# matajoh/fourier_feature_nets

Measured on AMD Instinct MI355X. Metric: rays/sec (train), higher is better.
Workload: dtype f32

## Files before the change

fourier_feature_nets_amd/csrc/fourier_features.h:

```cpp
#pragma once
#include "common.h"

namespace ffn {

typedef float f32x4 __attribute__((ext_vector_type(4)));

struct EncRegs {
    const float* tab;
    int F;
    int raw;
    float scale;
};

__device__ __forceinline__ EncRegs load_enc(const ffn_encoding& e, const float* table) {
    EncRegs r;
    r.F = e.num_freq;
    r.tab = table;
    r.raw = (e.include_input != 0 || e.num_freq == 0) ? 1 : 0;
    r.scale = e.scale;
    return r;
}

typedef ffn_f32x2 f32x2;

template <bool TRIG_ONLY>
__device__ __forceinline__ f32x4 feature_quad(const EncRegs& enc, int g, int h, float x0, float x1,
                                              float x2, f32x2 s0, f32x2 s1, f32x2 s2) {
    const int k = 4 * g + 2 * h;
    const int kk = TRIG_ONLY ? k : (k < kEncRowPitch - 2 ? k : kEncRowPitch - 2);
    const f32x2 b0 = *reinterpret_cast<const f32x2*>(enc.tab + kk);
    const f32x2 b1 = *reinterpret_cast<const f32x2*>(enc.tab + kEncRowPitch + kk);
    const f32x2 b2 = *reinterpret_cast<const f32x2*>(enc.tab + 2 * kEncRowPitch + kk);
    const f32x2 amp = *reinterpret_cast<const f32x2*>(enc.tab + 3 * kEncRowPitch + kk);
    f32x2 ang = b0 * s0;
    ang = __builtin_elementwise_fma(s1, b1, ang);
    ang = __builtin_elementwise_fma(s2, b2, ang);
    f32x2 sn, cs;
    fast_sincos_n<f32x2, 2>(ang, sn, cs);
    const f32x2 c = amp * cs, s = amp * sn;
    f32x4 v;
    if (TRIG_ONLY) {
        v[0] = c[0]; v[1] = s[0]; v[2] = c[1]; v[3] = s[1];
        return v;
    }
#pragma unroll
    for (int j = 0; j < 2; ++j) {
        const int off = 2 * (k + j - enc.F);
        const float raw_even = (enc.raw && off == 0) ? x0 : ((enc.raw && off == 2) ? x2 : 0.0f);
        const float raw_odd = (enc.raw && off == 0) ? x1 : 0.0f;
        const bool trig = k + j < enc.F;
        v[2 * j] = trig ? c[j] : raw_even;
        v[2 * j + 1] = trig ? s[j] : raw_odd;
    }
    return v;
}

__device__ __forceinline__ void feature_oct(const EncRegs& enc, int g, int h, f32x4 s0, f32x4 s1,
                                            f32x4 s2, f32x4& va, f32x4& vb) {
    const float* t = enc.tab + 4 * g + 2 * h;
    auto two = [](const float* p) {
        const f32x2 lo = *reinterpret_cast<const f32x2*>(p), hi = *reinterpret_cast<const f32x2*>(p + 4);
        f32x4 v; v[0] = lo[0]; v[1] = lo[1]; v[2] = hi[0]; v[3] = hi[1];
        return v;
    };
    const f32x4 b0 = two(t), b1 = two(t + kEncRowPitch), b2 = two(t + 2 * kEncRowPitch);
    const f32x4 amp = two(t + 3 * kEncRowPitch);
    f32x4 ang = b0 * s0;
    ang = __builtin_elementwise_fma(s1, b1, ang);
    ang = __builtin_elementwise_fma(s2, b2, ang);
    f32x4 sn, cs;
    fast_sincos_n<f32x4, 4>(ang, sn, cs);
    const f32x4 c = amp * cs, s = amp * sn;
    va[0] = c[0]; va[1] = s[0]; va[2] = c[1]; va[3] = s[1];
    vb[0] = c[2]; vb[1] = s[2]; vb[2] = c[3]; vb[3] = s[3];
}

}
```

fourier_feature_nets_amd/csrc/mlp.hip:

```cpp
#include "fourier_features.h"
#include "composite_terms.h"
#include "focus_terms.h"
#include "occupancy_map.h"

namespace ffn {

typedef float f32x4 __attribute__((ext_vector_type(4)));
typedef f32x4 __attribute__((address_space(3))) lds_f32x4;
__device__ __forceinline__ lds_f32x4* lds_slab(const char* generic_lds_address) {
    return (lds_f32x4*)(uint32_t)(uintptr_t)generic_lds_address;
}
typedef float f32x16 __attribute__((ext_vector_type(16)));

constexpr int kSamplesPerWave = 32;
constexpr int kWavesPerBlock = 4;
constexpr int kActBytesPerWave = 32 * 1024;
constexpr int kBiasLdsFloats = 4096;

enum Mode { kInfer = 0, kTrainFwd = 1, kBackward = 2 };

__global__ void __launch_bounds__(256)
pack_kernel(const float* __restrict__ src, int rows, int cols, int ld, int transpose,
            const int32_t* __restrict__ row_map, const int32_t* __restrict__ col_map, int groups,
            int tiles, float* __restrict__ dst) {
    const int64_t total = (int64_t)groups * tiles * 256;
    for (int64_t e = (int64_t)blockIdx.x * blockDim.x + threadIdx.x; e < total;
         e += (int64_t)gridDim.x * blockDim.x) {
        const int p = (int)(e & 3);
        const int lane = (int)((e >> 2) & 63);
        const int64_t go = e >> 8;
        const int o = (int)(go % tiles);
        const int g = (int)(go / tiles);
        int r = 32 * o + (lane & 31);
        int c = 8 * g + 4 * (lane >> 5) + p;
        if (row_map != nullptr) r = row_map[r];
// ... 22 lines not shown
    }
    const int64_t total = (int64_t)job.groups * job.tiles * 256;
    for (int64_t e = (int64_t)blockIdx.x * blockDim.x + threadIdx.x; e < total;
         e += (int64_t)gridDim.x * blockDim.x) {
        const int p = (int)(e & 3);
        const int lane = (int)((e >> 2) & 63);
        const int64_t go = e >> 8;
        const int o = (int)(go % job.tiles);
        const int g = (int)(go / job.tiles);
        const int r = 32 * o + (lane & 31);
        int c = 8 * g + 4 * (lane >> 5) + p;
        if (job.col_map != nullptr) c = job.col_map[c];
        float v = 0.0f;
        if (c >= 0) {
            const int sr = job.transpose ? c : r;
            const int sc = job.transpose ? r : c;
            if (sr < job.rows && sc < job.cols) v = job.src[(int64_t)sr * job.ld + sc];
        }
        job.dst[e] = v;
    }
}

template <bool SAVE>
__device__ __forceinline__ void generate_features(const EncRegs& enc, int c0, int count, int h,
                                                  int s, int lane, float x0, float x1, float x2,
                                                  lds_f32x4* act, f32x4* fsave, int g_begin, int g_step) {
    const f32x2 s0 = (f32x2)(enc.scale * x0), s1 = (f32x2)(enc.scale * x1), s2 = (f32x2)(enc.scale * x2);
    const f32x4 q0 = (f32x4)(enc.scale * x0), q1 = (f32x4)(enc.scale * x1), q2 = (f32x4)(enc.scale * x2);
    int g_trig = (enc.F >> 2) - c0;
    g_trig = g_trig < 0 ? 0 : (g_trig > count ? count : g_trig);
    g_trig &= ~3;
    for (int g = g_begin; g < count; g += g_step) {
        f32x4 v[4];
        if (g < g_trig) {
            feature_oct(enc, c0 + g, h, q0, q1, q2, v[0], v[1]);
            feature_oct(enc, c0 + g + 2, h, q0, q1, q2, v[2], v[3]);
        } else {
#pragma unroll
            for (int u = 0; u < 4; ++u) v[u] = feature_quad<false>(enc, c0 + g + u, h, x0, x1, x2, s0, s1, s2);
        }
#pragma unroll
        for (int u = 0; u < 4; ++u) {
            act[(g + u) * 64 + lane] = v[u];
            if (SAVE) __builtin_nontemporal_store(v[u], &fsave[(2 * (c0 + g + u) + h) * 32 + (s ^ ((2 * (c0 + g + u) + h) & 15))]);
        }
    }
}

template <int OT>
__device__ __forceinline__ void mma_group(f32x16 (&acc)[OT], const f32x4 (&a)[OT], f32x4 x) {
#pragma unroll
    for (int p = 0; p < 4; ++p)
#pragma unroll
        for (int o = 0; o < OT; ++o)
            acc[o] = __builtin_amdgcn_mfma_f32_32x32x2f32(a[o][p], x[p], acc[o], 0, 0, 0);
}

template <int OT>
__device__ __forceinline__ void pipeline_plain() {
    __builtin_amdgcn_sched_group_barrier(0x020, 2 * OT, 0);
    __builtin_amdgcn_sched_group_barrier(0x100, 2, 0);
    __builtin_amdgcn_sched_group_barrier(0x008, 8 * OT, 0);
}
template <int OT, bool SAVES = false>
__device__ __forceinline__ void pipeline_spread() {
    __builtin_amdgcn_sched_group_barrier(0x100, 2, 0);
    if (SAVES) __builtin_amdgcn_sched_group_barrier(0x040, 2, 0);
#pragma unroll
    for (int i = 0; i < 2 * OT; ++i) {
        __builtin_amdgcn_sched_group_barrier(0x008, 4, 0);
        __builtin_amdgcn_sched_group_barrier(0x020, 1, 0);
    }
}
template <int OT>
__device__ __forceinline__ void load_group(f32x4 (&a)[OT], const f32x4* __restrict__ wg, int lane) {
    typedef const f32x4 __attribute__((address_space(1)))* gptr;
    const gptr lo = (gptr)wg;
    gptr hi = (gptr)(wg + 4 * 64);
    if (OT > 4) asm volatile("" : "+s"(hi));
#pragma unroll
    for (int o = 0; o < OT; ++o) a[o] = (o < 4 ? lo : hi)[(o & 3) * 64 + lane];
}

struct WaveCtx {
    int lane, h, s;
    float x0, x1, x2;
    float v0, v1, v2;
    f32x4 dl;
    lds_f32x4* act;
    const float* enc_table;
    const float* bias_lds;
    const float* bias_glb;
    uint4* masks;
    int64_t block;
    int64_t num_blocks;
    int64_t slab_block0;
    int64_t slab_blocks;
    float logit[4];
    int half;
    bool active;
};

__device__ __forceinline__ int saved_index(int cq, int s) { return cq * 32 + (s ^ (cq & 15)); }

__device__ __forceinline__ f32x4* slab_block(const ffn_mlp_chain& ch, float* base, int slot,
                                             const WaveCtx& w) {
    return reinterpret_cast<f32x4*>(base + ch.slot_offset[slot] * w.slab_blocks * 32) +
           (w.slab_block0 + w.block) * (int64_t)(ch.slot_channels[slot] * 8);
}

__device__ __forceinline__ void team_barrier() {
    asm volatile("s_waitcnt lgkmcnt(0)" ::: "memory");
    __builtin_amdgcn_s_barrier();
}

template <int OT, int MODE, int TWP, int FLAV, bool BIG = false>
__device__ __forceinline__ void run_step(const ffn_mlp_chain& ch, const ffn_step& L,
                                         const ffn_step* next, WaveCtx& w,
                                         const float* __restrict__ packed_w,
                                         f32x4 (&pre)[16],
                                         float* __restrict__ slab_out) {
    constexpr bool WIDE = TWP > 1;
    constexpr int TW = TWP;
    constexpr int kChunk = BIG ? 128 : (WIDE ? 64 : 32);
    const int half = WIDE ? w.half : 0;
    f32x16 acc[OT];
    if (MODE == kBackward) {
#pragma unroll
        for (int o = 0; o < OT; ++o)
#pragma unroll
            for (int r = 0; r < 16; ++r) acc[o][r] = 0.0f;
    } else if (L.b_off + 32 * OT * TW <= kBiasLdsFloats) {
        const float* bv = w.bias_lds + L.b_off + 32 * OT * half + 4 * w.h;
#pragma unroll
        for (int o = 0; o < OT; ++o)
#pragma unroll
            for (int q = 0; q < 4; ++q) {
                const f32x4 b4 = *reinterpret_cast<const f32x4*>(bv + 32 * o + 8 * q);
#pragma unroll
                for (int p = 0; p < 4; ++p) acc[o][4 * q + p] = b4[p];
            }
    } else {
        const float* bv = w.bias_glb + L.b_off + 32 * OT * half + 4 * w.h;
#pragma unroll
        for (int o = 0; o < OT; ++o)
#pragma unroll
            for (int q = 0; q < 4; ++q) {
                const f32x4 b4 = *reinterpret_cast<const f32x4*>(bv + 32 * o + 8 * q);
#pragma unroll
                for (int p = 0; p < 4; ++p) acc[o][4 * q + p] = b4[p];
            }
    }

    const f32x4* wp = reinterpret_cast<const f32x4*>(packed_w + L.w_off) + half * OT * 64;
    const int GA = L.act_groups;
    const int GX = L.aux_groups;
    const int G = GA + GX;
    constexpr int kGroupStride = TW * OT * 64;
    f32x4 wa0[OT], wa1[OT], wb0[OT], wb1[OT];
    f32x4 x0, x1, x2, x3;
#pragma unroll
    for (int o = 0; o < OT; ++o) { wa0[o] = pre[o]; wa1[o] = pre[8 + o]; }
    int gnext = 2;
    const int glast = G - 2;
    const f32x4* wnext = wp + 2 * kGroupStride;
    const int64_t mask_at = (((int64_t)(L.mask_slot < 0 ? 0 : L.mask_slot) * w.num_blocks + w.block) * TW + half) * 64 + w.lane;
    uint4 mbits = make_uint4(0xffffffffu, 0xffffffffu, 0xffffffffu, 0xffffffffu);
    if (MODE == kBackward && L.mask_slot >= 0) mbits = w.masks[mask_at];

    constexpr bool kTripSaves = MODE == kTrainFwd && !WIDE;
    const int feat_chunks = MODE == kBackward ? 0 : (GX + kChunk - 1) / kChunk;
    const int segs = (GA > 0 ? 1 : 0) + feat_chunks;
    for (int sg = 0; sg < segs; ++sg) {
        const bool feat = !(GA > 0 && sg == 0);
        int count = GA;
        f32x4* save = nullptr;
        if (!feat) {
            if (kTripSaves || (MODE != kInfer && L.save_in_slot >= 0 && w.active))
                save = slab_block(ch, slab_out, L.save_in_slot, w);
        } else {
            const int c0 = (sg - (GA > 0 ? 1 : 0)) * kChunk;
            count = GX - c0 < kChunk ? GX - c0 : kChunk;
            const EncRegs enc = load_enc(ch.enc[L.enc_id], w.enc_table + L.enc_id * kEncTablePitch);
            const float p0 = L.enc_id == 0 ? w.x0 : w.v0;
            const float p1 = L.enc_id == 0 ? w.x1 : w.v1;
            const float p2 = L.enc_id == 0 ? w.x2 : w.v2;
            if (WIDE && sg > 0) team_barrier();
            if (kTripSaves) {
                generate_features<false>(enc, c0, count, w.h, w.s, w.lane, p0, p1, p2, w.act, nullptr,
                                         4 * half, 4 * TW);
                save = slab_block(ch, slab_out, L.save_enc_slot, w) + c0 * 64;
            } else if (MODE == kTrainFwd && L.save_enc_slot >= 0 && w.active) {
                generate_features<true>(enc, c0, count, w.h, w.s, w.lane, p0, p1, p2, w.act,
                                        slab_block(ch, slab_out, L.save_enc_slot, w), 4 * half, 4 * TW);
            } else {
                generate_features<false>(enc, c0, count, w.h, w.s, w.lane, p0, p1, p2, w.act, nullptr,
                                         4 * half, 4 * TW);
            }
            if (WIDE) team_barrier();
        }
        const bool saving = MODE != kInfer && save != nullptr;
        const bool save_0 = saving && (TW == 1 || half == 0);
        const bool save_1 = saving && (TW == 1 || half == (TW == 2 ? 0 : 1));
        const bool save_2 = saving && (TW == 1 || half == (TW == 2 ? 1 : 2));
        const bool save_3 = saving && (TW == 1 || half == (TW == 2 ? 1 : 3));
        const unsigned save_lane = (unsigned)(w.h * 512 + ((w.s ^ w.h) << 4));
        char* save_s = reinterpret_cast<char*>(save);
#define FFN_SAVE(g, value)                                                                     \
    __builtin_nontemporal_store((value), reinterpret_cast<f32x4*>(save_s + (int64_t)(g) * 1024 +   \
                              (save_lane ^ (unsigned)((((g) * 2) & 15) << 4))))
        const lds_f32x4* xa = w.act + w.lane;
        x0 = xa[0];
        x1 = xa[64];
        if (MODE == kInfer || kTripSaves) {
            for (int g = 0; g < count; g += 4) {
                load_group<OT>(wb0, wnext, w.lane);
                load_group<OT>(wb1, wnext + kGroupStride, w.lane);
                x2 = xa[128];
                x3 = xa[192];
// ... 57 lines not shown
        f32x4 d = w.dl;
        f32x4 sel;
#pragma unroll
        for (int p = 0; p < 4; ++p) {
            float v = 0.0f;
#pragma unroll
            for (int c = 0; c < 4; ++c) v = (c == L.lg_col + p && p < L.lg_n) ? d[c] : v;
            sel[p] = w.h == 0 ? v : 0.0f;
        }
        mma_group<OT>(acc, wa0, sel);
    }

    const int ot_next = next != nullptr ? next->out_tiles / TW : 0;
    const f32x4* wn = next != nullptr
        ? reinterpret_cast<const f32x4*>(packed_w + next->w_off) + half * ot_next * 64 + w.lane
        : nullptr;

    f32x4* save_out = nullptr;
    if (MODE != kInfer && L.save_out_slot >= 0 && w.active) save_out = slab_block(ch, slab_out, L.save_out_slot, w);
    const bool fused_head = FLAV == 0 ? (MODE != kBackward && L.head_off >= 0)
                                      : (MODE != kBackward && FLAV >= 2);
    const bool to_slab = FLAV == 0 ? L.dst == 0 : true;
    const bool save_y = FLAV == 0 ? save_out != nullptr : FLAV == 2;
    const float* head_base = BIG ? w.bias_glb : w.bias_lds;
    const float* hw = head_base + (fused_head ? L.head_off : 0) + 4 + 16 * w.h;
    if (fused_head && w.h == 0 && half == 0) {
        const f32x4 hb = *reinterpret_cast<const f32x4*>(head_base + L.head_off);
#pragma unroll
        for (int c = 0; c < 4; ++c) w.logit[c] += hb[c];
    }
    if (WIDE) team_barrier();
    int e_lane = w.lane, e_h = w.h, e_s = w.s;
    if (WIDE) asm volatile("" : "+v"(e_lane), "+v"(e_h), "+v"(e_s));
    unsigned sign_bits[4] = {0u, 0u, 0u, 0u};
    const int relu_floor = L.relu ? 0 : (int)0x80000000;
#pragma unroll
    for (int o = 0; o < 8; ++o) {
        if (o < ot_next) {
            pre[o] = wn[o * 64];
            pre[8 + o] = wn[(int64_t)(TW * ot_next + o) * 64];
        }
        if (o >= OT) continue;
#pragma unroll
        for (int q = 0; q < 4; ++q) {
            const int group = 4 * (OT * half + o) + q;
            f32x4 y;
            if (MODE == kBackward) {
                const unsigned word = o < 2 ? mbits.x : (o < 4 ? mbits.y : (o < 6 ? mbits.z : mbits.w));
#pragma unroll
                for (int p = 0; p < 4; ++p) {
                    const int filled = ((OT & 1) && o == OT - 1) ? 16 : 32;
                    const int bit = filled - 1 - (16 * (o & 1) + 4 * q + p);
                    const int keep = ((int)(word << (31 - bit))) >> 31;
                    const float a = acc[o][4 * q + p];
                    y[p] = __builtin_bit_cast(float, __builtin_bit_cast(int, a) & keep);
                }
                w.act[group * 64 + e_lane] = y;
                if (save_y) __builtin_nontemporal_store(y, &save_out[saved_index(2 * group + e_h, e_s)]);
            } else {
                f32x4 hw4[4];
                if (fused_head) {
#pragma unroll
                    for (int p = 0; p < 4; ++p) hw4[p] = *reinterpret_cast<const f32x4*>(hw + group * 32 + p * 4);
                }
#pragma unroll
                for (int p = 0; p < 4; ++p) {
                    float t = acc[o][4 * q + p];
                    if (MODE == kTrainFwd)
                        sign_bits[o >> 1] = __builtin_amdgcn_alignbit(sign_bits[o >> 1],
                                                                      __builtin_bit_cast(unsigned, 0.0f - t), 31);
                    y[p] = __builtin_bit_cast(float, __builtin_elementwise_max(__builtin_bit_cast(int, t), relu_floor));
                }
                if (to_slab) {
                    w.act[group * 64 + e_lane] = y;
                    if (fused_head) {
#pragma unroll
                        for (int p = 0; p < 4; ++p) {
#pragma unroll
                            for (int c = 0; c < 4; ++c) w.logit[c] = __builtin_fmaf(y[p], hw4[p][c], w.logit[c]);
                        }
                        if (MODE == kTrainFwd && save_y) __builtin_nontemporal_store(y, &save_out[saved_index(2 * group + e_h, e_s)]);
                    }
                } else if (!WIDE && o == 0 && q == 0) {
#pragma unroll
                    for (int c = 0; c < 4; ++c) {
                        const int p = c - L.out_col;
// ... 41 lines not shown
                else run_step<8, MODE, TWP, 1, BIG>(ch, L, next, w, packed_w, pre, slab_out);
            } else if (!head && L.dst == 0) run_step<8, MODE, TWP, 1, BIG>(ch, L, next, w, packed_w, pre, slab_out);
            else run_step<8, MODE, TWP, 0, BIG>(ch, L, next, w, packed_w, pre, slab_out);
        } else if ((TWP < 4 || BIG) && ot == 4) run_step<4, MODE, TWP, 0, BIG>(ch, L, next, w, packed_w, pre, slab_out);
        else if (ot == 2) run_step<2, MODE, TWP, 0, BIG>(ch, L, next, w, packed_w, pre, slab_out);
        else run_step<1, MODE, TWP, 0, BIG>(ch, L, next, w, packed_w, pre, slab_out);
    }
}

constexpr int kTeamScratchBytes = 3072;

template <int TWP>
__device__ __forceinline__ void wave_setup(WaveCtx& w, char* smem, int64_t n, int64_t& stride) {
    constexpr bool WIDE = TWP > 1;
    w.lane = threadIdx.x & 63;
    w.h = w.lane >> 5;
    w.s = w.lane & 31;
    const int wave_in_block = __builtin_amdgcn_readfirstlane(threadIdx.x >> 6);
    const int teams = kWavesPerBlock / TWP;
    const int team = wave_in_block / TWP;
    w.half = WIDE ? (wave_in_block % TWP) : 0;
    stride = (int64_t)gridDim.x * teams;
    w.act = lds_slab(smem + team * (kActBytesPerWave * kWavesPerBlock / teams));
    w.enc_table = reinterpret_cast<const float*>(smem + kWavesPerBlock * kActBytesPerWave);
    w.bias_lds = reinterpret_cast<const float*>(smem + kWavesPerBlock * kActBytesPerWave + kEncTableBytes);
    w.num_blocks = (n + kSamplesPerWave - 1) / kSamplesPerWave;
    w.block = (int64_t)blockIdx.x * teams + team;
    w.slab_block0 = 0;
    w.slab_blocks = w.num_blocks;
    w.active = true;
}

template <int MODE, int TWP, bool BIG = false>
__global__ void __launch_bounds__(256, 1)
mlp_forward_kernel(const ffn_mlp_chain ch, const float* __restrict__ packed_w,
                   const float* __restrict__ bias, const float* __restrict__ positions,
                   const float* __restrict__ views, int64_t n, float* __restrict__ logits,
                   float* __restrict__ saved, uint32_t* __restrict__ masks, int64_t slab_block0,
                   int64_t slab_blocks) {
    extern __shared__ __attribute__((aligned(16))) char smem[];
    stage_encoding_tables(ch.enc, reinterpret_cast<float*>(smem + kWavesPerBlock * kActBytesPerWave),
                          threadIdx.x, 256);
    {
        float* bl = reinterpret_cast<float*>(smem + kWavesPerBlock * kActBytesPerWave + kEncTableBytes);
        const int staged = ch.bias_floats < kBiasLdsFloats ? ch.bias_floats : kBiasLdsFloats;
        for (int i = threadIdx.x; i < staged; i += 256) bl[i] = bias[i];
    }
    __syncthreads();
    constexpr bool WIDE = TWP > 1;
    WaveCtx w;
    int64_t stride;
    wave_setup<TWP>(w, smem, n, stride);
    w.bias_glb = bias;
    if (slab_blocks > 0) { w.slab_block0 = slab_block0; w.slab_blocks = slab_blocks; }
    w.masks = reinterpret_cast<uint4*>(masks);
    f32x4* scratch = reinterpret_cast<f32x4*>(smem + kWavesPerBlock * kActBytesPerWave + kEncTableBytes +
                                              kBiasLdsFloats * 4) + ((threadIdx.x >> 6) / TWP) * (TWP - 1) * 64;
    const int64_t passes = WIDE ? (w.num_blocks + stride - 1) / stride : 0;
    const int64_t first = w.block;
    float in_next[6] = {0.f, 0.f, 0.f, 0.f, 0.f, 0.f};
    auto request_inputs = [&](int64_t block) {
        block = block < w.num_blocks ? block : w.num_blocks - 1;
        const int64_t sample = block * kSamplesPerWave + w.s;
        const int64_t src = sample < n ? sample : n - 1;
        in_next[0] = positions[src * 3 + 0]; in_next[1] = positions[src * 3 + 1]; in_next[2] = positions[src * 3 + 2];
        if (views != nullptr) {
            in_next[3] = views[src * 3 + 0]; in_next[4] = views[src * 3 + 1]; in_next[5] = views[src * 3 + 2];
        }
    };
    request_inputs(first);
    for (int64_t pass = 0; WIDE ? pass < passes : w.block < w.num_blocks; ++pass) {
        if (WIDE) {
            w.block = first + pass * stride;
            w.active = w.block < w.num_blocks;
            if (!w.active) w.block = w.num_blocks - 1;
        }
// ... 29 lines not shown
    const uint32_t* occ_bits; GridMap map;
    float* color; float* alpha; float* depth; int32_t* nan_flag;
    uint8_t* image; int64_t pixel_offset;
};

constexpr int kRenderScratchBytes = 4096;

template <bool WIDE>
__global__ void __launch_bounds__(256, 1)
render_fused_kernel(const ffn_mlp_chain ch, const float* __restrict__ packed_w,
                    const float* __restrict__ bias, const RenderParams p) {
    extern __shared__ __attribute__((aligned(16))) char smem[];
    stage_encoding_tables(ch.enc, reinterpret_cast<float*>(smem + kWavesPerBlock * kActBytesPerWave),
                          threadIdx.x, 256);
    {
        float* bl = reinterpret_cast<float*>(smem + kWavesPerBlock * kActBytesPerWave + kEncTableBytes);
        const int staged = ch.bias_floats < kBiasLdsFloats ? ch.bias_floats : kBiasLdsFloats;
        for (int i = threadIdx.x; i < staged; i += 256) bl[i] = bias[i];
    }
    __syncthreads();
    WaveCtx w;
    int64_t stride;
    wave_setup<(WIDE ? 2 : 1)>(w, smem, kSamplesPerWave, stride);
    w.bias_glb = bias;
    w.block = 0;
    w.masks = nullptr;
    const int wave_in_block = __builtin_amdgcn_readfirstlane(threadIdx.x >> 6);
    constexpr int kTeams = WIDE ? 2 : kWavesPerBlock;
    const int team = WIDE ? wave_in_block >> 1 : wave_in_block;
    char* scratch = smem + kWavesPerBlock * kActBytesPerWave + kEncTableBytes + kBiasLdsFloats * 4;
    f32x4* partial = reinterpret_cast<f32x4*>(scratch) + team * 64;
    uint16_t* slots = reinterpret_cast<uint16_t*>(scratch + (WIDE ? 2048 : 0)) + team * 256;
    volatile int* team_blocks = reinterpret_cast<volatile int*>(scratch + 3072);
    const int S = p.S;
    const int rays_per_round = gridDim.x * kTeams;
    const int rounds = (p.num_rays + rays_per_round - 1) / rays_per_round;
    for (int round = 0; round < rounds; ++round) {
        const int r = WIDE ? (round * (int)gridDim.x + (int)blockIdx.x) * 2 + team
                           : (int)blockIdx.x * kWavesPerBlock + team + round * rays_per_round;
        bool have = r < p.num_rays;
        const int rr = have ? r : 0;
        const int64_t ray = p.ray_index != nullptr ? p.ray_index[rr] : p.ray_base + rr;
        if (have && p.valid != nullptr && p.valid[ray] == 0) {
            if (w.lane == 0 && w.half == 0) {
                if (p.color != nullptr) {
                    p.color[(int64_t)r * 3 + 0] = 0.f; p.color[(int64_t)r * 3 + 1] = 0.f;
                    p.color[(int64_t)r * 3 + 2] = 0.f;
                }
                if (p.alpha != nullptr) p.alpha[r] = 0.f;
                if (p.depth != nullptr) p.depth[r] = 0.f;
            }
            have = false;
        }
        if (!WIDE && !have) continue;
        const float sx = p.starts[ray * 3 + 0], sy = p.starts[ray * 3 + 1], sz = p.starts[ray * 3 + 2];
        const float dx = p.dirs[ray * 3 + 0], dy = p.dirs[ray * 3 + 1], dz = p.dirs[ray * 3 + 2];
// ... 92 lines not shown

struct FocusParams {
    const float* starts; const float* dirs; const float* near_far; int64_t total_rays;
    const int64_t* ray_index; int num_rays; int S; int n_focus;
    const float* unit_focus; const float* u; float* t_io;
};

template <bool WIDE>
__global__ void __launch_bounds__(256, 1)
focus_fused_kernel(const ffn_mlp_chain ch, const float* __restrict__ packed_w,
                   const float* __restrict__ bias, const FocusParams p) {
    extern __shared__ __attribute__((aligned(16))) char smem[];
    stage_encoding_tables(ch.enc, reinterpret_cast<float*>(smem + kWavesPerBlock * kActBytesPerWave),
                          threadIdx.x, 256);
    {
        float* bl = reinterpret_cast<float*>(smem + kWavesPerBlock * kActBytesPerWave + kEncTableBytes);
        const int staged = ch.bias_floats < kBiasLdsFloats ? ch.bias_floats : kBiasLdsFloats;
        for (int i = threadIdx.x; i < staged; i += 256) bl[i] = bias[i];
    }
    __syncthreads();
    WaveCtx w;
    int64_t stride;
    wave_setup<(WIDE ? 2 : 1)>(w, smem, kSamplesPerWave, stride);
    w.bias_glb = bias;
    w.block = 0;
    w.masks = nullptr;
    const int wave_in_block = __builtin_amdgcn_readfirstlane(threadIdx.x >> 6);
    constexpr int kTeams = WIDE ? 2 : kWavesPerBlock;
    const int team = WIDE ? wave_in_block >> 1 : wave_in_block;
    f32x4* partial = reinterpret_cast<f32x4*>(smem + kWavesPerBlock * kActBytesPerWave + kEncTableBytes +
                                              kBiasLdsFloats * 4) + team * 64;
    const int teams = gridDim.x * kTeams;
    const int n = p.n_focus;
    const int nblk = (n + 31) >> 5;
    const int rounds = (p.num_rays + teams - 1) / teams;
    for (int round = 0; round < rounds; ++round) {
        const int r0 = round * teams + (int)blockIdx.x * kTeams + team;
        const bool have = r0 < p.num_rays;
        if (!WIDE && !have) continue;
        const int r = have ? r0 : 0;
        const int64_t ray = p.ray_index[r];
        const float sx = p.starts[ray * 3 + 0], sy = p.starts[ray * 3 + 1], sz = p.starts[ray * 3 + 2];
        const float dx = p.dirs[ray * 3 + 0], dy = p.dirs[ray * 3 + 1], dz = p.dirs[ray * 3 + 2];
        const float near = p.near_far[ray], far = p.near_far[p.total_rays + ray];
        const float span = sub_rn(far, near);
        auto t_of = [&](int j) -> float { return mul_add_rn(p.unit_focus[j], span, near); };
        float sigma_logit = 0.0f;
// ... 298 lines not shown
```

fourier_feature_nets_amd/mlp_engine.py:

```python

import ctypes
import os
from typing import Dict, List, Optional, Sequence

import torch

from . import _lib
from ._lib import c_i, c_i64
from .ops import _call, _dev

MAX_STEPS = 16
BIAS_LDS_FLOATS = 4096
WGRAD_GROUPS = 256
UNIT_COST = {4: 24, 2: 13, 1: 8}
HEAD_COST = 5
FOLD_COST = {(2, 2): 7, (2, 4): 5, (1, 2): 4, (1, 4): 3}
if os.environ.get("FFN_FOLD_COST"):
    _c = [int(v) for v in os.environ["FFN_FOLD_COST"].split(",")]
    FOLD_COST = {(2, 2): _c[0], (2, 4): _c[1], (1, 2): _c[2], (1, 4): _c[3]}
UNIT_COST16 = {4: 24, 2: 24, 1: 20}
HEAD_COST16 = 13
if os.environ.get("FFN_UNIT_COST16"):
    _c = [int(v) for v in os.environ["FFN_UNIT_COST16"].split(",")]
    UNIT_COST16, HEAD_COST16 = {4: _c[0], 2: _c[1], 1: _c[2]}, _c[3]
UNIT_COST_X6 = {4: 24, 2: 17, 1: 17}
HEAD_COST_X6 = 10
if os.environ.get("FFN_UNIT_COST_X6"):
    _c = [int(v) for v in os.environ["FFN_UNIT_COST_X6"].split(",")]
    UNIT_COST_X6, HEAD_COST_X6 = {4: _c[0], 2: _c[1], 1: _c[2]}, _c[3]
if os.environ.get("FFN_UNIT_COST"):
    _c = [int(v) for v in os.environ["FFN_UNIT_COST"].split(",")]
    UNIT_COST, HEAD_COST = {4: _c[0], 2: _c[1], 1: _c[2]}, _c[3]


TAIL_PAIRS = os.environ.get("FFN_TAIL_PAIRS", "1") == "1"
TAIL_QUADS = os.environ.get("FFN_TAIL_QUADS", "1") == "1"
TAIL_MAX_FULL_ROUNDS = 16


class FfnEncoding(ctypes.Structure):
    _fields_ = [("b", ctypes.c_void_p), ("a", ctypes.c_void_p), ("num_freq", ctypes.c_int32),
                ("include_input", ctypes.c_int32), ("scale", ctypes.c_float),
                ("width", ctypes.c_int32)]


class FfnStep(ctypes.Structure):
    _fields_ = [("act_groups", ctypes.c_int32), ("aux_groups", ctypes.c_int32),
                ("enc_id", ctypes.c_int32), ("lg_col", ctypes.c_int32), ("lg_n", ctypes.c_int32),
                ("out_tiles", ctypes.c_int32), ("relu", ctypes.c_int32), ("dst", ctypes.c_int32),
                ("out_col", ctypes.c_int32), ("out_n", ctypes.c_int32),
                ("save_in_slot", ctypes.c_int32), ("save_out_slot", ctypes.c_int32),
                ("mask_slot", ctypes.c_int32), ("save_enc_slot", ctypes.c_int32),
                ("head_off", ctypes.c_int32), ("out_slot", ctypes.c_int32),
                ("w_off", ctypes.c_int64), ("b_off", ctypes.c_int64)]


class FfnMlpChain(ctypes.Structure):
    _fields_ = [("enc", FfnEncoding * 2), ("step", FfnStep * MAX_STEPS),
                ("num_steps", ctypes.c_int32), ("num_slots", ctypes.c_int32),
                ("bias_floats", ctypes.c_int32), ("wide", ctypes.c_int32),
                ("slot_channels", ctypes.c_int32 * MAX_STEPS),
                ("slot_offset", ctypes.c_int64 * MAX_STEPS)]


class FfnWgradUnit(ctypes.Structure):
    _fields_ = [("m_slot", ctypes.c_int32), ("m_cq0", ctypes.c_int32), ("m_quads", ctypes.c_int32),
# ... 53 lines not shown
    return host.to(device)


class EncodingSpec:

    def __init__(self, b: Optional[torch.Tensor], a: Optional[torch.Tensor], scale: float,
                 include_input: bool, device: Optional[torch.device] = None, num_inputs: int = 3):
        if num_inputs not in (1, 2, 3):
            raise NotImplementedError("encodings of 1, 2 or 3 inputs (got %d)" % num_inputs)
        self.num_inputs = int(num_inputs)
        self.num_freq = 0 if b is None else int(b.shape[1])
        dev = device if device is not None else (b.device if b is not None else None)
        if b is None:
            b = torch.zeros((3, 1), dtype=torch.float32, device=dev)
        elif b.shape[0] != num_inputs:
            raise ValueError("B has %d rows for %d inputs" % (b.shape[0], num_inputs))
        elif num_inputs < 3:
            b = torch.cat([b, torch.zeros((3 - num_inputs, b.shape[1]), dtype=b.dtype,
                                          device=b.device)])
        if a is None:
            a = torch.ones((max(self.num_freq, 1),), dtype=torch.float32, device=dev)
        self.b = b.contiguous()
        self.a = a.contiguous()
        self.scale = float(scale)
        self.include_input = bool(include_input) or self.num_freq == 0
        if self.num_freq > 256:
            raise NotImplementedError("encodings with more than 256 frequencies")
        natural = 2 * self.num_freq + (self.num_inputs if self.include_input else 0)
        self.natural_width = natural
        self.width = ((natural + 31) // 32) * 32

    def natural_index(self, internal: int) -> int:
        freq = self.num_freq
        if internal < 2 * freq:
            k = internal >> 1
            return k if (internal & 1) == 0 else freq + k
        if self.include_input and internal < 2 * freq + self.num_inputs:
            return internal
        return -1


class DenseSpec:

    def __init__(self, weight, bias, act_in: int, enc_id: Optional[int], relu: bool,
                 to_logits: Optional[tuple] = None):
        self.weight = weight
# ... 87 lines not shown
        self._build_pair_chains()

    def _dz_buffer(self, floats: int) -> torch.Tensor:
        buf = getattr(self, "_dz", None)
        if buf is None or buf.numel() < floats:
            self._dz = buf = None
            self._dz = buf = torch.empty((floats + floats // 16,), dtype=torch.float32,
                                         device=self.device)
        return buf[:floats]

    def release_workspaces(self):
        self._dz = None
        self._workspaces.clear()

    def _fill_encodings(self, chain):
        for i, enc in enumerate(self.encodings):
            e = chain.enc[i]
            e.b = enc.b.data_ptr()
            e.a = enc.a.data_ptr()
            e.num_freq = enc.num_freq
            e.include_input = 1 if enc.include_input else 0
            e.scale = enc.scale
            e.width = enc.width
        for i in range(len(self.encodings), 2):
            src = chain.enc[0]
            chain.enc[i].b, chain.enc[i].a = src.b, src.a
            chain.enc[i].num_freq, chain.enc[i].include_input = src.num_freq, src.include_input
            chain.enc[i].scale, chain.enc[i].width = src.scale, src.width

    def _build_forward(self):
        fwd = FfnMlpChain()
        self._fill_encodings(fwd)
        widest = max([sp.out for sp in self.layers if sp.to_logits is None] or [0])
        self.wide = widest > 256
        self.big = widest > 512
        self.wide_level = 3 if self.big else (1 if self.wide else 0)
        fwd.wide = self.wide_level
        producer = -1
        for i, sp in enumerate(self.layers):
            sp.act_in_p = self.layers[producer].out_p if (sp.act_in > 0 and producer >= 0) else sp.act_in
            if sp.to_logits is None:
                sp.out_p = _padded_width(sp.out, self.wide_level)
                producer = i
        w_off = b_off = h_off = 0
        self.col_maps: List[torch.Tensor] = []
        self.step_of: List[Optional[int]] = []
        self.fwd_shapes: Dict[int, tuple] = {}
        self.fused_heads = []
# ... 767 lines not shown
```

fourier_feature_nets_amd/models.py:

```python

import math
import os
from typing import List, Optional, Sequence

import torch
import torch.nn as nn

from .mlp_engine import DenseSpec, EncodingSpec, MlpProgram
from .sampler import _notice_once


class _FusedChainFunction(torch.autograd.Function):

    @staticmethod
    def forward(ctx, module, grad_mode, positions, views, *params):
        prog = module.program()
        if grad_mode and (positions.requires_grad or (views is not None and views.requires_grad)):
            raise NotImplementedError(
                "gradients w.r.t. sample positions / view directions are not produced by the "
                "fused kernels (the volume-rendering path never needs them); detach the inputs")
        positions = positions.contiguous()
        views = None if views is None else views.contiguous()
        track = grad_mode and any(ctx.needs_input_grad[4:])
        saved = None
# ... 61 lines not shown
        self.precision = self.train_precision = mode
        self._precision_is_default = mode != "f32"

    def effective_precision(self, mode: str) -> str:
        if mode == "f32" or not self._precision_is_default or self.program().covers(mode):
            return mode
        _notice_once("%s: no %s kernels for this chain (%s) -- it runs in exact f32"
                     % (type(self).__name__, mode,
                        "layers wider than 256 channels" if mode == "bf16x6" else "unfused logits heads"))
        return "f32"

    def _chain(self, device):
        raise NotImplementedError

    def _dense_params(self) -> List[nn.Parameter]:
        raise NotImplementedError

    def invalidate_packed(self):
        self._packed_key = None

    def load_state_dict(self, *args, **kwargs):
        out = super().load_state_dict(*args, **kwargs)
        self.invalidate_packed()
        return out

    def check_params(self, device: torch.device):
        params = self._dense_params()
        for k in range(0, len(params), 2):
            w, b = params[k], params[k + 1]
            for name, t in (("weight", w), ("bias", b)):
                if t.device != device:
                    raise RuntimeError("%s: a dense %s lives on %s, the model on %s; move it with "
                                       "the model (.to(device)) before calling it"
                                       % (type(self).__name__, name, t.device, device))
                if t.dtype != torch.float32:
                    raise TypeError("%s: a dense %s is %s; the kernels take float32"
                                    % (type(self).__name__, name, t.dtype))
            if w.dim() != 2 or w.stride(1) != 1:
                raise ValueError("%s: a dense weight must be a row-major (out, in) matrix, got "
                                 "shape %s" % (type(self).__name__, tuple(w.shape)))
            if b.dim() > 1 or b.numel() != w.shape[0] or not b.is_contiguous():
                raise ValueError("%s: a bias of shape %s for a layer of %d outputs (a (%d,) or, "
                                 "for one output, a 0-d tensor)"
                                 % (type(self).__name__, tuple(b.shape), w.shape[0], w.shape[0]))

    def program(self) -> MlpProgram:
# ... 244 lines not shown
```

include/ffn_hip.h:

```cpp
#ifndef FFN_HIP_H
#define FFN_HIP_H

#include <stdint.h>

#ifdef __cplusplus
extern "C" {
#endif

#define FFN_ABI_VERSION 3

int ffn_abi_version(void);
const char* ffn_last_error_string(void);

int ffn_raygen_nearfar(const float* unproj, const float* cam_pos, const float* points,
                       int num_cameras, int width, int height, const float* box_lo,
                       const float* box_hi,
                       float* starts, float* directions, float* near_far, uint8_t* valid,
                       void* stream);

int ffn_sample_t(const float* near_far, int64_t num_rays_total, const int64_t* ray_index,
                 int num_rays, int count, const float* unit, const float* noise,
                 float anneal, float* t_out, int t_stride, void* stream);

int ffn_materialise_samples(const float* starts, const float* directions,
// ... 57 lines not shown
                        int32_t* nan_flag, void* stream);

int ffn_loss_from_partials(const float* partials, int num_blocks, float colour_count,
                           float alpha_count, float alpha_weight, float* sums, float* loss_out,
                           void* stream);

int ffn_loss_value(const float* sums, float colour_count, float alpha_count, float alpha_weight,
                   float* loss_out, void* stream);

int ffn_to_image(const float* colors, const int64_t* pixel_index, int64_t n, int width,
                 int height, uint8_t* image, void* stream);

int ffn_ycrcb_to_rgb_u8(uint8_t* image, int64_t pixels, void* stream);

#define FFN_MAX_STEPS 16

typedef struct ffn_encoding {
    const float* b;
    const float* a;
    int32_t num_freq;
    int32_t include_input;
    float scale;
    int32_t width;
} ffn_encoding;

typedef struct ffn_step {
    int32_t act_groups;
    int32_t aux_groups;
    int32_t enc_id;
    int32_t lg_col;
    int32_t lg_n;
    int32_t out_tiles;
    int32_t relu;
    int32_t dst;
    int32_t out_col;
    int32_t out_n;
    int32_t save_in_slot;
    int32_t save_out_slot;
    int32_t mask_slot;
    int32_t save_enc_slot;
    int32_t head_off;
    int32_t out_slot;
    int64_t w_off;
    int64_t b_off;
} ffn_step;

// ... 440 lines not shown
```

Before: 1.539 million.

## Software-pipeline Fourier feature generation, skip unit amplitudes, use explicit LDS address spaces

Splits feature generation into a trig-only burst loop that reads the next octet's encoding table entries and computes its angles while the current octet's sincos and stores run, with a scheduling barrier to group the LDS reads. When all encoding amplitudes are exactly one (detected on the host), the amplitude loads and multiplies are dropped. Pointers to the encoding table and bias are retyped to explicit LDS or global address spaces so the compiler emits ds/global loads instead of flat ones. This adds register pressure from the lookahead and an ABI change to the encoding struct.

```diff
diff --git a/fourier_feature_nets_amd/csrc/fourier_features.h b/fourier_feature_nets_amd/csrc/fourier_features.h
--- a/fourier_feature_nets_amd/csrc/fourier_features.h
+++ b/fourier_feature_nets_amd/csrc/fourier_features.h
@@ -4,34 +4,38 @@
 namespace ffn {
 
 typedef float f32x4 __attribute__((ext_vector_type(4)));
+typedef ffn_f32x2 f32x2;
+typedef const float __attribute__((address_space(3))) lds_cfloat;
+typedef const f32x2 __attribute__((address_space(3))) lds_cf32x2;
 
 struct EncRegs {
-    const float* tab;
+    lds_cfloat* tab;
     int F;
     int raw;
+    int unit_amp;
     float scale;
 };
 
-__device__ __forceinline__ EncRegs load_enc(const ffn_encoding& e, const float* table) {
+__device__ __forceinline__ EncRegs load_enc(const ffn_encoding& e, lds_cfloat* table) {
     EncRegs r;
     r.F = e.num_freq;
     r.tab = table;
     r.raw = (e.include_input != 0 || e.num_freq == 0) ? 1 : 0;
+    r.unit_amp = e.unit_amp;
     r.scale = e.scale;
     return r;
 }
-
-typedef ffn_f32x2 f32x2;
 
 template <bool TRIG_ONLY>
 __device__ __forceinline__ f32x4 feature_quad(const EncRegs& enc, int g, int h, float x0, float x1,
                                               float x2, f32x2 s0, f32x2 s1, f32x2 s2) {
     const int k = 4 * g + 2 * h;
     const int kk = TRIG_ONLY ? k : (k < kEncRowPitch - 2 ? k : kEncRowPitch - 2);
-    const f32x2 b0 = *reinterpret_cast<const f32x2*>(enc.tab + kk);
-    const f32x2 b1 = *reinterpret_cast<const f32x2*>(enc.tab + kEncRowPitch + kk);
-    const f32x2 b2 = *reinterpret_cast<const f32x2*>(enc.tab + 2 * kEncRowPitch + kk);
-    const f32x2 amp = *reinterpret_cast<const f32x2*>(enc.tab + 3 * kEncRowPitch + kk);
+    lds_cfloat* t = enc.tab + kk;
+    const f32x2 b0 = *reinterpret_cast<lds_cf32x2*>(t);
+    const f32x2 b1 = *reinterpret_cast<lds_cf32x2*>(t + kEncRowPitch);
+    const f32x2 b2 = *reinterpret_cast<lds_cf32x2*>(t + 2 * kEncRowPitch);
+    const f32x2 amp = *reinterpret_cast<lds_cf32x2*>(t + 3 * kEncRowPitch);
     f32x2 ang = b0 * s0;
     ang = __builtin_elementwise_fma(s1, b1, ang);
     ang = __builtin_elementwise_fma(s2, b2, ang);
@@ -55,22 +59,32 @@
     return v;
 }
 
-__device__ __forceinline__ void feature_oct(const EncRegs& enc, int g, int h, f32x4 s0, f32x4 s1,
-                                            f32x4 s2, f32x4& va, f32x4& vb) {
-    const float* t = enc.tab + 4 * g + 2 * h;
-    auto two = [](const float* p) {
-        const f32x2 lo = *reinterpret_cast<const f32x2*>(p), hi = *reinterpret_cast<const f32x2*>(p + 4);
+struct OctTab { f32x4 b0, b1, b2, amp; };
+
+template <bool UNIT>
+__device__ __forceinline__ OctTab read_oct(lds_cfloat* t) {
+    auto two = [](lds_cfloat* p) {
+        const f32x2 lo = *reinterpret_cast<lds_cf32x2*>(p), hi = *reinterpret_cast<lds_cf32x2*>(p + 4);
         f32x4 v; v[0] = lo[0]; v[1] = lo[1]; v[2] = hi[0]; v[3] = hi[1];
         return v;
     };
-    const f32x4 b0 = two(t), b1 = two(t + kEncRowPitch), b2 = two(t + 2 * kEncRowPitch);
-    const f32x4 amp = two(t + 3 * kEncRowPitch);
-    f32x4 ang = b0 * s0;
-    ang = __builtin_elementwise_fma(s1, b1, ang);
-    ang = __builtin_elementwise_fma(s2, b2, ang);
+    OctTab o;
+    o.b0 = two(t); o.b1 = two(t + kEncRowPitch); o.b2 = two(t + 2 * kEncRowPitch);
+    o.amp = UNIT ? (f32x4)(1.0f) : two(t + 3 * kEncRowPitch);
+    return o;
+}
+
+__device__ __forceinline__ f32x4 oct_angles(const OctTab& o, f32x4 s0, f32x4 s1, f32x4 s2) {
+    f32x4 ang = o.b0 * s0;
+    ang = __builtin_elementwise_fma(s1, o.b1, ang);
+    return __builtin_elementwise_fma(s2, o.b2, ang);
+}
+
+template <bool UNIT>
+__device__ __forceinline__ void feature_oct(f32x4 ang, f32x4 amp, f32x4& va, f32x4& vb) {
     f32x4 sn, cs;
     fast_sincos_n<f32x4, 4>(ang, sn, cs);
-    const f32x4 c = amp * cs, s = amp * sn;
+    const f32x4 c = UNIT ? cs : amp * cs, s = UNIT ? sn : amp * sn;
     va[0] = c[0]; va[1] = s[0]; va[2] = c[1]; va[3] = s[1];
     vb[0] = c[2]; vb[1] = s[2]; vb[2] = c[3]; vb[3] = s[3];
 }
diff --git a/fourier_feature_nets_amd/csrc/mlp.hip b/fourier_feature_nets_amd/csrc/mlp.hip
--- a/fourier_feature_nets_amd/csrc/mlp.hip
+++ b/fourier_feature_nets_amd/csrc/mlp.hip
@@ -11,6 +11,9 @@
     return (lds_f32x4*)(uint32_t)(uintptr_t)generic_lds_address;
 }
 typedef float f32x16 __attribute__((ext_vector_type(16)));
+typedef const f32x4 __attribute__((address_space(3))) lds_cf32x4;
+typedef const float __attribute__((address_space(1))) glb_cfloat;
+typedef const f32x4 __attribute__((address_space(1))) glb_cf32x4;
 
 constexpr int kSamplesPerWave = 32;
 constexpr int kWavesPerBlock = 4;
@@ -79,6 +82,51 @@
 }
 
 template <bool SAVE>
+__device__ __forceinline__ void store_features(const f32x4 (&v)[4], int c0, int g, int h, int s, int lane,
+                                               lds_f32x4* act, f32x4* fsave) {
+#pragma unroll
+    for (int u = 0; u < 4; ++u) {
+        act[(g + u) * 64 + lane] = v[u];
+        if (SAVE) __builtin_nontemporal_store(v[u], &fsave[(2 * (c0 + g + u) + h) * 32 + (s ^ ((2 * (c0 + g + u) + h) & 15))]);
+    }
+}
+
+template <bool SAVE, bool UNIT, bool AHEAD>
+__device__ __forceinline__ void generate_oct_trips(const EncRegs& enc, int c0, int g_trig, int h, int s,
+                                                   int lane, f32x4 q0, f32x4 q1, f32x4 q2, lds_f32x4* act,
+                                                   f32x4* fsave, int& g, int g_step) {
+    if (g >= g_trig) return;
+    lds_cfloat* t0 = enc.tab + 4 * c0 + 2 * h;
+    if (!AHEAD) {
+        for (; g < g_trig; g += g_step) {
+            const OctTab a = read_oct<UNIT>(t0 + 4 * g), b = read_oct<UNIT>(t0 + 4 * g + 8);
+            f32x4 v[4];
+            feature_oct<UNIT>(oct_angles(a, q0, q1, q2), a.amp, v[0], v[1]);
+            feature_oct<UNIT>(oct_angles(b, q0, q1, q2), b.amp, v[2], v[3]);
+            store_features<SAVE>(v, c0, g, h, s, lane, act, fsave);
+        }
+        return;
+    }
+    OctTab a = read_oct<UNIT>(t0 + 4 * g), b = read_oct<UNIT>(t0 + 4 * g + 8);
+    f32x4 ang_a = oct_angles(a, q0, q1, q2), ang_b = oct_angles(b, q0, q1, q2);
+    f32x4 amp_a = a.amp, amp_b = b.amp;
+    for (; g < g_trig; g += g_step) {
+        lds_cfloat* tn = t0 + 4 * (g + g_step < g_trig ? g + g_step : g);
+        a = read_oct<UNIT>(tn);
+        b = read_oct<UNIT>(tn + 8);
+        f32x4 v[4];
+        feature_oct<UNIT>(ang_a, amp_a, v[0], v[1]);
+        feature_oct<UNIT>(ang_b, amp_b, v[2], v[3]);
+        store_features<SAVE>(v, c0, g, h, s, lane, act, fsave);
+        ang_a = oct_angles(a, q0, q1, q2);
+        ang_b = oct_angles(b, q0, q1, q2);
+        amp_a = a.amp;
+        amp_b = b.amp;
+        __builtin_amdgcn_sched_group_barrier(0x100, UNIT ? 6 : 8, 0);
+    }
+}
+
+template <bool SAVE, bool AHEAD>
 __device__ __forceinline__ void generate_features(const EncRegs& enc, int c0, int count, int h,
                                                   int s, int lane, float x0, float x1, float x2,
                                                   lds_f32x4* act, f32x4* fsave, int g_begin, int g_step) {
@@ -87,20 +135,14 @@
     int g_trig = (enc.F >> 2) - c0;
     g_trig = g_trig < 0 ? 0 : (g_trig > count ? count : g_trig);
     g_trig &= ~3;
-    for (int g = g_begin; g < count; g += g_step) {
+    int g = g_begin;
+    if (enc.unit_amp) generate_oct_trips<SAVE, true, AHEAD>(enc, c0, g_trig, h, s, lane, q0, q1, q2, act, fsave, g, g_step);
+    else generate_oct_trips<SAVE, false, AHEAD>(enc, c0, g_trig, h, s, lane, q0, q1, q2, act, fsave, g, g_step);
+    for (; g < count; g += g_step) {
         f32x4 v[4];
-        if (g < g_trig) {
-            feature_oct(enc, c0 + g, h, q0, q1, q2, v[0], v[1]);
-            feature_oct(enc, c0 + g + 2, h, q0, q1, q2, v[2], v[3]);
-        } else {
-#pragma unroll
-            for (int u = 0; u < 4; ++u) v[u] = feature_quad<false>(enc, c0 + g + u, h, x0, x1, x2, s0, s1, s2);
-        }
-#pragma unroll
-        for (int u = 0; u < 4; ++u) {
-            act[(g + u) * 64 + lane] = v[u];
-            if (SAVE) __builtin_nontemporal_store(v[u], &fsave[(2 * (c0 + g + u) + h) * 32 + (s ^ ((2 * (c0 + g + u) + h) & 15))]);
-        }
+#pragma unroll
+        for (int u = 0; u < 4; ++u) v[u] = feature_quad<false>(enc, c0 + g + u, h, x0, x1, x2, s0, s1, s2);
+        store_features<SAVE>(v, c0, g, h, s, lane, act, fsave);
     }
 }
 
@@ -145,9 +187,9 @@
     float v0, v1, v2;
     f32x4 dl;
     lds_f32x4* act;
-    const float* enc_table;
-    const float* bias_lds;
-    const float* bias_glb;
+    lds_cfloat* enc_table;
+    lds_cfloat* bias_lds;
+    glb_cfloat* bias_glb;
     uint4* masks;
     int64_t block;
     int64_t num_blocks;
@@ -188,22 +230,22 @@
 #pragma unroll
             for (int r = 0; r < 16; ++r) acc[o][r] = 0.0f;
     } else if (L.b_off + 32 * OT * TW <= kBiasLdsFloats) {
-        const float* bv = w.bias_lds + L.b_off + 32 * OT * half + 4 * w.h;
+        lds_cfloat* bv = w.bias_lds + L.b_off + 32 * OT * half + 4 * w.h;
 #pragma unroll
         for (int o = 0; o < OT; ++o)
 #pragma unroll
             for (int q = 0; q < 4; ++q) {
-                const f32x4 b4 = *reinterpret_cast<const f32x4*>(bv + 32 * o + 8 * q);
+                const f32x4 b4 = *reinterpret_cast<lds_cf32x4*>(bv + 32 * o + 8 * q);
 #pragma unroll
                 for (int p = 0; p < 4; ++p) acc[o][4 * q + p] = b4[p];
             }
     } else {
-        const float* bv = w.bias_glb + L.b_off + 32 * OT * half + 4 * w.h;
+        glb_cfloat* bv = w.bias_glb + L.b_off + 32 * OT * half + 4 * w.h;
 #pragma unroll
         for (int o = 0; o < OT; ++o)
 #pragma unroll
             for (int q = 0; q < 4; ++q) {
-                const f32x4 b4 = *reinterpret_cast<const f32x4*>(bv + 32 * o + 8 * q);
+                const f32x4 b4 = *reinterpret_cast<glb_cf32x4*>(bv + 32 * o + 8 * q);
 #pragma unroll
                 for (int p = 0; p < 4; ++p) acc[o][4 * q + p] = b4[p];
             }
@@ -244,14 +286,14 @@
             const float p2 = L.enc_id == 0 ? w.x2 : w.v2;
             if (WIDE && sg > 0) team_barrier();
             if (kTripSaves) {
-                generate_features<false>(enc, c0, count, w.h, w.s, w.lane, p0, p1, p2, w.act, nullptr,
+                generate_features<false, !WIDE>(enc, c0, count, w.h, w.s, w.lane, p0, p1, p2, w.act, nullptr,
                                          4 * half, 4 * TW);
                 save = slab_block(ch, slab_out, L.save_enc_slot, w) + c0 * 64;
             } else if (MODE == kTrainFwd && L.save_enc_slot >= 0 && w.active) {
-                generate_features<true>(enc, c0, count, w.h, w.s, w.lane, p0, p1, p2, w.act,
+                generate_features<true, !WIDE>(enc, c0, count, w.h, w.s, w.lane, p0, p1, p2, w.act,
                                         slab_block(ch, slab_out, L.save_enc_slot, w), 4 * half, 4 * TW);
             } else {
-                generate_features<false>(enc, c0, count, w.h, w.s, w.lane, p0, p1, p2, w.act, nullptr,
+                generate_features<false, !WIDE>(enc, c0, count, w.h, w.s, w.lane, p0, p1, p2, w.act, nullptr,
                                          4 * half, 4 * TW);
             }
             if (WIDE) team_barrier();
@@ -355,10 +397,13 @@
                                       : (MODE != kBackward && FLAV >= 2);
     const bool to_slab = FLAV == 0 ? L.dst == 0 : true;
     const bool save_y = FLAV == 0 ? save_out != nullptr : FLAV == 2;
-    const float* head_base = BIG ? w.bias_glb : w.bias_lds;
-    const float* hw = head_base + (fused_head ? L.head_off : 0) + 4 + 16 * w.h;
+    auto head_read = [&](int at) -> f32x4 {
+        if (BIG) return *reinterpret_cast<glb_cf32x4*>(w.bias_glb + at);
+        return *reinterpret_cast<lds_cf32x4*>(w.bias_lds + at);
+    };
+    const int hw = (fused_head ? L.head_off : 0) + 4 + 16 * w.h;
     if (fused_head && w.h == 0 && half == 0) {
-        const f32x4 hb = *reinterpret_cast<const f32x4*>(head_base + L.head_off);
+        const f32x4 hb = head_read(L.head_off);
 #pragma unroll
         for (int c = 0; c < 4; ++c) w.logit[c] += hb[c];
     }
@@ -394,7 +439,7 @@
                 f32x4 hw4[4];
                 if (fused_head) {
 #pragma unroll
-                    for (int p = 0; p < 4; ++p) hw4[p] = *reinterpret_cast<const f32x4*>(hw + group * 32 + p * 4);
+                    for (int p = 0; p < 4; ++p) hw4[p] = head_read(hw + group * 32 + p * 4);
                 }
 #pragma unroll
                 for (int p = 0; p < 4; ++p) {
@@ -482,8 +527,8 @@
     w.half = WIDE ? (wave_in_block % TWP) : 0;
     stride = (int64_t)gridDim.x * teams;
     w.act = lds_slab(smem + team * (kActBytesPerWave * kWavesPerBlock / teams));
-    w.enc_table = reinterpret_cast<const float*>(smem + kWavesPerBlock * kActBytesPerWave);
-    w.bias_lds = reinterpret_cast<const float*>(smem + kWavesPerBlock * kActBytesPerWave + kEncTableBytes);
+    w.enc_table = (lds_cfloat*)(lds_slab(smem) + kWavesPerBlock * kActBytesPerWave / 16);
+    w.bias_lds = w.enc_table + kEncTableBytes / 4;
     w.num_blocks = (n + kSamplesPerWave - 1) / kSamplesPerWave;
     w.block = (int64_t)blockIdx.x * teams + team;
     w.slab_block0 = 0;
@@ -511,7 +556,7 @@
     WaveCtx w;
     int64_t stride;
     wave_setup<TWP>(w, smem, n, stride);
-    w.bias_glb = bias;
+    w.bias_glb = (glb_cfloat*)bias;
     if (slab_blocks > 0) { w.slab_block0 = slab_block0; w.slab_blocks = slab_blocks; }
     w.masks = reinterpret_cast<uint4*>(masks);
     f32x4* scratch = reinterpret_cast<f32x4*>(smem + kWavesPerBlock * kActBytesPerWave + kEncTableBytes +
@@ -587,7 +632,7 @@
     WaveCtx w;
     int64_t stride;
     wave_setup<(WIDE ? 2 : 1)>(w, smem, kSamplesPerWave, stride);
-    w.bias_glb = bias;
+    w.bias_glb = (glb_cfloat*)bias;
     w.block = 0;
     w.masks = nullptr;
     const int wave_in_block = __builtin_amdgcn_readfirstlane(threadIdx.x >> 6);
@@ -596,7 +641,9 @@
     char* scratch = smem + kWavesPerBlock * kActBytesPerWave + kEncTableBytes + kBiasLdsFloats * 4;
     f32x4* partial = reinterpret_cast<f32x4*>(scratch) + team * 64;
     uint16_t* slots = reinterpret_cast<uint16_t*>(scratch + (WIDE ? 2048 : 0)) + team * 256;
-    volatile int* team_blocks = reinterpret_cast<volatile int*>(scratch + 3072);
+    typedef volatile int __attribute__((address_space(3))) lds_vint;
+    lds_vint* team_blocks = (lds_vint*)(lds_slab(smem) + (kWavesPerBlock * kActBytesPerWave + kEncTableBytes +
+                                                          kBiasLdsFloats * 4 + 3072) / 16);
     const int S = p.S;
     const int rays_per_round = gridDim.x * kTeams;
     const int rounds = (p.num_rays + rays_per_round - 1) / rays_per_round;
@@ -735,7 +782,7 @@
     WaveCtx w;
     int64_t stride;
     wave_setup<(WIDE ? 2 : 1)>(w, smem, kSamplesPerWave, stride);
-    w.bias_glb = bias;
+    w.bias_glb = (glb_cfloat*)bias;
     w.block = 0;
     w.masks = nullptr;
     const int wave_in_block = __builtin_amdgcn_readfirstlane(threadIdx.x >> 6);
diff --git a/fourier_feature_nets_amd/mlp_engine.py b/fourier_feature_nets_amd/mlp_engine.py
--- a/fourier_feature_nets_amd/mlp_engine.py
+++ b/fourier_feature_nets_amd/mlp_engine.py
@@ -36,12 +36,14 @@
 TAIL_PAIRS = os.environ.get("FFN_TAIL_PAIRS", "1") == "1"
 TAIL_QUADS = os.environ.get("FFN_TAIL_QUADS", "1") == "1"
 TAIL_MAX_FULL_ROUNDS = 16
+UNIT_AMP_BURSTS = os.environ.get("FFN_GENERIC_BURSTS", "0") != "1"
 
 
 class FfnEncoding(ctypes.Structure):
     _fields_ = [("b", ctypes.c_void_p), ("a", ctypes.c_void_p), ("num_freq", ctypes.c_int32),
                 ("include_input", ctypes.c_int32), ("scale", ctypes.c_float),
-                ("width", ctypes.c_int32)]
+                ("width", ctypes.c_int32), ("unit_amp", ctypes.c_int32),
+                ("reserved", ctypes.c_int32)]
 
 
 class FfnStep(ctypes.Structure):
@@ -141,6 +143,7 @@
             a = torch.ones((max(self.num_freq, 1),), dtype=torch.float32, device=dev)
         self.b = b.contiguous()
         self.a = a.contiguous()
+        self.unit_amp = bool((self.a == 1.0).all().item())
         self.scale = float(scale)
         self.include_input = bool(include_input) or self.num_freq == 0
         if self.num_freq > 256:
@@ -274,8 +277,10 @@
             e.include_input = 1 if enc.include_input else 0
             e.scale = enc.scale
             e.width = enc.width
+            e.unit_amp = 1 if (UNIT_AMP_BURSTS and enc.unit_amp) else 0
         for i in range(len(self.encodings), 2):
             src = chain.enc[0]
+            chain.enc[i].unit_amp = src.unit_amp
             chain.enc[i].b, chain.enc[i].a = src.b, src.a
             chain.enc[i].num_freq, chain.enc[i].include_input = src.num_freq, src.include_input
             chain.enc[i].scale, chain.enc[i].width = src.scale, src.width
diff --git a/fourier_feature_nets_amd/models.py b/fourier_feature_nets_amd/models.py
--- a/fourier_feature_nets_amd/models.py
+++ b/fourier_feature_nets_amd/models.py
@@ -107,6 +107,7 @@
     def load_state_dict(self, *args, **kwargs):
         out = super().load_state_dict(*args, **kwargs)
         self.invalidate_packed()
+        self._prog = None
         return out
 
     def check_params(self, device: torch.device):
diff --git a/include/ffn_hip.h b/include/ffn_hip.h
--- a/include/ffn_hip.h
+++ b/include/ffn_hip.h
@@ -103,6 +103,8 @@
     int32_t include_input;
     float scale;
     int32_t width;
+    int32_t unit_amp;
+    int32_t reserved;
 } ffn_encoding;
 
 typedef struct ffn_step {
```

After: 1.540 million (median of 2 runs). About the same (+0.1%).
